# jcyk/gtos

Measured on AMD Instinct MI355X. Metric: graphs/sec training step (100-node AMR, batch 64), higher is better.
Workload: dtype bf16

## Files before the change

gtos_amd/csrc/rel_attn.hip:

```cpp
#include "common.h"
#include "attn_tile.h"
#include <cstdlib>
#include <type_traits>

namespace {

template <typename T> struct Raw8;
template <> struct Raw8<bf16_t> {
    uint4 a;
    __device__ __forceinline__ void load(const bf16_t* p) { a = *reinterpret_cast<const uint4*>(p); }
    __device__ __forceinline__ void zero() { a = make_uint4(0, 0, 0, 0); }
    __device__ __forceinline__ void get(float (&v)[8]) const {
        v[0] = lo_bf(a.x); v[1] = hi_bf(a.x); v[2] = lo_bf(a.y); v[3] = hi_bf(a.y);
        v[4] = lo_bf(a.z); v[5] = hi_bf(a.z); v[6] = lo_bf(a.w); v[7] = hi_bf(a.w);
    }
};
template <> struct Raw8<float> {
    float4 a, b;
    __device__ __forceinline__ void load(const float* p) {
        a = *reinterpret_cast<const float4*>(p); b = *reinterpret_cast<const float4*>(p + 4);
    }
    __device__ __forceinline__ void zero() { a = make_float4(0, 0, 0, 0); b = a; }
    __device__ __forceinline__ void get(float (&v)[8]) const {
        v[0] = a.x; v[1] = a.y; v[2] = a.z; v[3] = a.w; v[4] = b.x; v[5] = b.y; v[6] = b.z; v[7] = b.w;
    }
};

#ifndef GTOS_ATTN_U
#define GTOS_ATTN_U 1
#endif
template <typename T> struct Unroll { static constexpr int U = GTOS_ATTN_U; };
template <> struct Unroll<float> { static constexpr int U = 1; };

struct AttnArgs {
    const void *q, *k, *v; int64_t ldq, ldk, ldv;
    const void* rel;
    const int* idx_q;
    const int* idx_k;
    const uint8_t* key_pad;
    const uint8_t* attn_mask;
    void* o; int64_t ldo;
    float* lse;
    float* w;
    const void* d_o; int64_t lddo;
    const float* dw;
    void *dq, *dk, *dv; int64_t lddq, lddk, lddv;
    int64_t ld_drel;
    void* d_rel;
    float* pd;
    float* gs;
    int T, S, B, H, d, mode;
    int hd, nhs, lr;
    float scale, p_drop; uint64_t seed;
};

struct LaneMap { int LR, g, cl, c, h; bool act, lead; };
template <int LH, bool GEN>
__device__ __forceinline__ LaneMap lane_map(int d, int H, int hd, int nhs, int lr, int lane) {
    LaneMap m;
    if constexpr (!GEN) {
        m.LR = d >> 3; m.g = lane / m.LR; m.cl = lane % m.LR; m.c = m.cl * 8; m.h = m.cl / LH;
        m.act = true; m.lead = (m.cl % LH) == 0;
    } else {
        m.LR = lr; m.g = lane / lr; m.cl = lane % lr;
        const int hl = m.cl / LH, p = m.cl % LH;
        m.h = (int)blockIdx.y * nhs + hl;
        m.c = m.h * hd + p * 8;
        m.act = m.h < H && p * 8 < hd;
        m.lead = m.act && p == 0;
    }
    return m;
}

#define GTOS_DPP(v, ctrl) __builtin_bit_cast(float, __builtin_amdgcn_update_dpp(0, __builtin_bit_cast(int, (v)), (ctrl), 0xF, 0xF, true))
template <int LH> __device__ __forceinline__ float head_sum(float v) {
    if (LH >= 2) v += GTOS_DPP(v, 0xB1);
    if (LH >= 4) v += GTOS_DPP(v, 0x4E);
    if (LH >= 8) v += GTOS_DPP(v, 0x141);
    if (LH >= 16) v += GTOS_DPP(v, 0x140);
    if (LH >= 32) v += __shfl_xor(v, 16);
    if (LH >= 64) v += __shfl_xor(v, 32);
    return v;
}

__device__ __forceinline__ bool map_block(int rows, int B, int& row, int& b) {
    const int blk = blockIdx.x;
    if ((B & 7) == 0) { const int x = blk & 7, w = blk >> 3, gpx = B >> 3; b = x * gpx + (w % gpx); row = w / gpx; }
    else { b = blk % B; row = blk / B; }
    return row < rows;
}

__device__ __forceinline__ bool is_masked(const AttnArgs& a, int i, int j, int b) {
    bool m = false;
    if (a.key_pad) m = a.key_pad[(int64_t)j * a.B + b] != 0;
    if (a.attn_mask) m = m || (a.attn_mask[(int64_t)i * a.S + j] != 0);
    return m;
}

constexpr int MAXS_LDS = 1024;
__device__ __forceinline__ const unsigned char* stage_mask(const AttnArgs& a, int i, int b, unsigned char* sm) {
    const bool use = (a.key_pad || a.attn_mask) && a.S <= MAXS_LDS;
    if (use) for (int j = threadIdx.x; j < a.S; j += 256) sm[j] = is_masked(a, i, j, b) ? 1 : 0;
    __syncthreads();
    return use ? sm : nullptr;
}
__device__ __forceinline__ const int* stage_ids(const int* __restrict__ src, int n, int* sid) {
    if (!src || n > MAXS_LDS) return nullptr;
    for (int j = threadIdx.x; j < n; j += 256) sid[j] = src[j];
    return sid;
}
__device__ __forceinline__ bool key_dead(const AttnArgs& a, const unsigned char* sm, int i, int j, int b) {
    if (sm) return sm[j] != 0;
    return (a.key_pad || a.attn_mask) ? is_masked(a, i, j, b) : false;
}

template <typename T, int LH, bool GEN>
__global__ __launch_bounds__(256, 4) void rel_attn_fwd_kernel(AttnArgs a) {
    if (a.p_drop > 0.f) a.seed = live_seed(a.seed);
    constexpr int U = Unroll<T>::U;
    __shared__ unsigned char smask[MAXS_LDS];
    __shared__ int sid[MAXS_LDS];
    __shared__ float red[4][64][10];
    __shared__ float fin[64][2];
    int i, b;
    if (!map_block(a.T, a.B, i, b)) return;
    const int* sidp = stage_ids(a.mode == 2 ? a.idx_q + ((int64_t)i * a.B + b) * a.S : nullptr, a.S, sid);
    const unsigned char* sm = stage_mask(a, i, b, smask);
    const int lane = threadIdx.x & 63, wv = threadIdx.x >> 6;
    const LaneMap lm = lane_map<LH, GEN>(a.d, a.H, a.hd, a.nhs, a.lr, lane);
    const int d = a.d, LR = lm.LR, G = 64 / LR, g = lm.g, c = lm.c, h = lm.h;
    const bool act = lm.act, lead = lm.lead;
    const int KS = 4 * G;
    const T* qp = static_cast<const T*>(a.q) + ((int64_t)i * a.B + b) * a.ldq + c;
    const T* kb = static_cast<const T*>(a.k) + (int64_t)b * a.ldk + c;
    const T* vb = static_cast<const T*>(a.v) + (int64_t)b * a.ldv + c;
    const T* rel = static_cast<const T*>(a.rel);
    const int* iq = a.mode == 2 ? (sidp ? sidp : a.idx_q + ((int64_t)i * a.B + b) * a.S) : nullptr;
    const float keep_scale = a.p_drop > 0.f ? 1.f / (1.f - a.p_drop) : 1.f;
    const int joff = wv * G + g;

    float qf[8];
    { Raw8<T> r; r.zero(); if (act) r.load(qp); r.get(qf); }
    float m = -INFINITY, l = 0.f, o[8] = {0, 0, 0, 0, 0, 0, 0, 0};

    struct KeySet { Raw8<T> ra[U], rb[U], k[U], v[U]; int tn[U]; };
    auto load_idx = [&](int jb, KeySet& ks) {
#pragma unroll
        for (int u = 0; u < U; ++u) { const int j = jb + u * KS + joff; ks.tn[u] = (iq && j < a.S) ? iq[j] : 0; }
    };
    auto issue = [&](int jb, KeySet& ks) {
#pragma unroll
        for (int u = 0; u < U; ++u) {
            const int j = jb + u * KS + joff;
            ks.ra[u].zero(); ks.rb[u].zero(); ks.k[u].zero(); ks.v[u].zero();
            if (j < a.S && act) {
                ks.k[u].load(kb + (int64_t)j * a.B * a.ldk);
                ks.v[u].load(vb + (int64_t)j * a.B * a.ldv);
                if (a.mode == 1) {
                    const T* p = rel + (((int64_t)j * a.T + i) * a.B + b) * (2 * d) + c;
                    ks.ra[u].load(p); ks.rb[u].load(p + d);
                } else if (a.mode == 2) {
                    const T* p = rel + (int64_t)(ks.tn[u] & 0x7fffffff) * (2 * d) + c;
                    ks.ra[u].load(p); ks.rb[u].load(p + d);
                }
            }
        }
    };
    auto consume = [&](int jb, const KeySet& ks) {
#pragma unroll
        for (int u = 0; u < U; ++u) {
            const int j = jb + u * KS + joff;
            float ra[8], rb[8], kf[8], vf[8];
            ks.ra[u].get(ra); ks.rb[u].get(rb); ks.k[u].get(kf); ks.v[u].get(vf);
            float s = 0.f;
#pragma unroll
            for (int e = 0; e < 8; ++e) s = fmaf(qf[e] + ra[e], kf[e] + rb[e], s);
            s = head_sum<LH>(s) * a.scale;
            const bool dead = (j >= a.S) || key_dead(a, sm, i, j, b);
            if (dead) s = -INFINITY;
            if (a.w && j < a.S && lead) a.w[(((int64_t)i * a.S + j) * a.B + b) * a.H + h] = s;
            const float mn = fmaxf(m, s);
            float alpha = 1.f, pe = 0.f;
            if (mn != -INFINITY) { alpha = __expf(m - mn); pe = __expf(s - mn); }
            l = l * alpha + pe;
            float pv = pe;
            if (a.p_drop > 0.f && !dead)
                pv = drop_keep(a.seed, (((uint64_t)i * a.S + j) * a.B + b) * a.H + h, a.p_drop) ? pe * keep_scale : 0.f;
#pragma unroll
            for (int e = 0; e < 8; ++e) o[e] = fmaf(o[e], alpha, pv * vf[e]);
            m = mn;
        }
    };
    const int STEP = KS * U;
    KeySet A, Bs;
    load_idx(0, A); load_idx(STEP, Bs);
    issue(0, A);
    for (int jb = 0; jb < a.S; jb += 2 * STEP) {
        issue(jb + STEP, Bs); load_idx(jb + 2 * STEP, A);
        consume(jb, A);
        if (jb + STEP >= a.S) break;
        issue(jb + 2 * STEP, A); load_idx(jb + 3 * STEP, Bs);
        consume(jb + STEP, Bs);
    }
    for (int off = LR; off < 64; off <<= 1) {
        const float m2 = __shfl_xor(m, off), l2 = __shfl_xor(l, off);
        const float mn = fmaxf(m, m2);
        float a1 = 1.f, a2 = 1.f;
        if (mn != -INFINITY) { a1 = __expf(m - mn); a2 = __expf(m2 - mn); }
        l = l * a1 + l2 * a2;
#pragma unroll
        for (int e = 0; e < 8; ++e) { const float o2 = __shfl_xor(o[e], off); o[e] = o[e] * a1 + o2 * a2; }
        m = mn;
    }
    red[wv][lane][0] = m; red[wv][lane][1] = l;
#pragma unroll
    for (int e = 0; e < 8; ++e) red[wv][lane][2 + e] = o[e];
    __syncthreads();
    if (wv == 0) {
#pragma unroll
        for (int w2 = 1; w2 < 4; ++w2) {
            const float m2 = red[w2][lane][0], l2 = red[w2][lane][1];
            const float mn = fmaxf(m, m2);
            float a1 = 1.f, a2 = 1.f;
            if (mn != -INFINITY) { a1 = __expf(m - mn); a2 = __expf(m2 - mn); }
            l = l * a1 + l2 * a2;
#pragma unroll
            for (int e = 0; e < 8; ++e) o[e] = o[e] * a1 + red[w2][lane][2 + e] * a2;
            m = mn;
        }
        const float inv = l > 0.f ? 1.f / l : 0.f;
        fin[lane][0] = m; fin[lane][1] = inv;
        if (g == 0 && act) {
            float r[8];
#pragma unroll
            for (int e = 0; e < 8; ++e) r[e] = o[e] * inv;
            Vec8<T>::store(static_cast<T*>(a.o) + ((int64_t)i * a.B + b) * a.ldo + c, r);
            if (lead) a.lse[((int64_t)i * a.B + b) * a.H + h] = (l > 0.f) ? m + __logf(l) : -INFINITY;
        }
    }
    if (a.w) {
        __syncthreads();
        if (lead) {
            const float mf = fin[lane][0], inv = fin[lane][1];
            for (int j = joff; j < a.S; j += KS) {
                const int64_t off = (((int64_t)i * a.S + j) * a.B + b) * a.H + h;
                const float s = a.w[off];
                float p = (s == -INFINITY || inv <= 0.f) ? 0.f : __expf(s - mf) * inv;
                if (a.p_drop > 0.f && p > 0.f) p = drop_keep(a.seed, (uint64_t)off, a.p_drop) ? p * keep_scale : 0.f;
                a.w[off] = p;
            }
        }
    }
}

template <typename T, int LH, bool GEN>
__global__ __launch_bounds__(256) void rel_attn_bwd_q_kernel(AttnArgs a) {
    if (a.p_drop > 0.f) a.seed = live_seed(a.seed);
    constexpr int U = Unroll<T>::U;
    __shared__ unsigned char smask[MAXS_LDS];
    __shared__ int sid[MAXS_LDS];
    __shared__ float red[4][64][8];
    __shared__ float redw[4][64];
    int i, b;
    if (!map_block(a.T, a.B, i, b)) return;
    const int* sidp = stage_ids(a.mode == 2 ? a.idx_q + ((int64_t)i * a.B + b) * a.S : nullptr, a.S, sid);
    const unsigned char* sm = stage_mask(a, i, b, smask);
    const int lane = threadIdx.x & 63, wv = threadIdx.x >> 6;
    const LaneMap lm = lane_map<LH, GEN>(a.d, a.H, a.hd, a.nhs, a.lr, lane);
    const int d = a.d, LR = lm.LR, G = 64 / LR, g = lm.g, c = lm.c, h = lm.h;
    const bool act = lm.act, lead = lm.lead;
    const int KS = 4 * G, joff = wv * G + g;
    const int64_t row = (int64_t)i * a.B + b;
    const T* kb = static_cast<const T*>(a.k) + (int64_t)b * a.ldk + c;
    const T* vb = static_cast<const T*>(a.v) + (int64_t)b * a.ldv + c;
    const T* rel = static_cast<const T*>(a.rel);
    const int* iq = a.mode == 2 ? (sidp ? sidp : a.idx_q + row * a.S) : nullptr;
    const float keep_scale = a.p_drop > 0.f ? 1.f / (1.f - a.p_drop) : 1.f;

    float qf[8], dof[8], of[8];
    { Raw8<T> r; r.zero(); if (act) r.load(static_cast<const T*>(a.q) + row * a.ldq + c); r.get(qf); }
    { Raw8<T> r; r.zero(); if (act) r.load(static_cast<const T*>(a.d_o) + row * a.lddo + c); r.get(dof); }
    { Raw8<T> r; r.zero(); if (act) r.load(static_cast<const T*>(a.o) + row * a.ldo + c); r.get(of); }
    float D = 0.f;
#pragma unroll
    for (int e = 0; e < 8; ++e) D = fmaf(dof[e], of[e], D);
    D = head_sum<LH>(D);
    if (a.dw) {
        float acc = 0.f;
        for (int j = joff; j < a.S && act; j += KS) {
            const int64_t off = (((int64_t)i * a.S + j) * a.B + b) * a.H + h;
            acc = fmaf(a.w[off], a.dw[off], acc);
        }
        for (int off = LR; off < 64; off <<= 1) acc += __shfl_xor(acc, off);
        redw[wv][lane] = acc;
        __syncthreads();
        D += redw[0][lane] + redw[1][lane] + redw[2][lane] + redw[3][lane];
    }
    const float lse = act ? a.lse[row * a.H + h] : -INFINITY;
    float dq[8] = {0, 0, 0, 0, 0, 0, 0, 0};

    struct KeySet { Raw8<T> ra[U], rb[U], k[U], v[U]; int tn[U], tw[U]; };
    auto load_idx = [&](int jb, KeySet& ks) {
#pragma unroll
        for (int u = 0; u < U; ++u) { const int j = jb + u * KS + joff; ks.tn[u] = (iq && j < a.S) ? iq[j] : 0; }
    };
    auto issue = [&](int jb, KeySet& ks) {
#pragma unroll
        for (int u = 0; u < U; ++u) {
            const int j = jb + u * KS + joff;
            ks.ra[u].zero(); ks.rb[u].zero(); ks.k[u].zero(); ks.v[u].zero();
            if (j < a.S && act) {
                ks.k[u].load(kb + (int64_t)j * a.B * a.ldk);
                ks.v[u].load(vb + (int64_t)j * a.B * a.ldv);
                if (a.mode == 1) {
                    const T* p = rel + (((int64_t)j * a.T + i) * a.B + b) * (2 * d) + c;
                    ks.ra[u].load(p); ks.rb[u].load(p + d);
                } else if (a.mode == 2) {
                    const T* p = rel + (int64_t)(ks.tn[u] & 0x7fffffff) * (2 * d) + c;
                    ks.ra[u].load(p); ks.rb[u].load(p + d);
                    ks.tw[u] = ks.tn[u];
                }
            }
        }
    };
    auto consume = [&](int jb, const KeySet& ks) {
#pragma unroll
        for (int u = 0; u < U; ++u) {
            const int j = jb + u * KS + joff;
            if (j >= a.S) continue;
            float ra[8], rb[8], kf[8], vf[8];
            ks.ra[u].get(ra); ks.rb[u].get(rb); ks.k[u].get(kf); ks.v[u].get(vf);
            float s = 0.f, dpv = 0.f;
#pragma unroll
            for (int e = 0; e < 8; ++e) {
                ra[e] += qf[e]; rb[e] += kf[e];
                s = fmaf(ra[e], rb[e], s);
                dpv = fmaf(dof[e], vf[e], dpv);
            }
            s = head_sum<LH>(s) * a.scale;
            dpv = head_sum<LH>(dpv);
            const int64_t off = (((int64_t)i * a.S + j) * a.B + b) * a.H + h;
            const bool dead = key_dead(a, sm, i, j, b) || lse == -INFINITY;
            const float p = dead ? 0.f : __expf(s - lse);
            float keep = 1.f;
            if (a.p_drop > 0.f) keep = drop_keep(a.seed, (uint64_t)off, a.p_drop) ? keep_scale : 0.f;
            float dp = dpv;
            if (a.dw && act) dp += a.dw[off];
            const float gsc = a.scale * p * (keep * dp - D);
            if (lead) { a.pd[off] = p * keep; a.gs[off] = gsc; }
            float dra[8], drb[8];
#pragma unroll
            for (int e = 0; e < 8; ++e) { dra[e] = gsc * rb[e]; drb[e] = gsc * ra[e]; dq[e] += dra[e]; }
            if (!act) {
            } else if (a.mode == 1) {
                T* p2 = static_cast<T*>(a.d_rel) + (((int64_t)j * a.T + i) * a.B + b) * (2 * d) + c;
                Vec8<T>::store(p2, dra);
                Vec8<T>::store(p2 + d, drb);
            } else if (a.mode == 2 && ks.tw[u] < 0 && a.d_rel) {
                T* p2 = static_cast<T*>(a.d_rel) + (int64_t)(ks.tw[u] & 0x7fffffff) * a.ld_drel + c;
                Vec8<T>::store(p2, dra);
                Vec8<T>::store(p2 + d, drb);
            }
        }
    };
    const int STEP = KS * U;
    KeySet A, Bs;
    load_idx(0, A); load_idx(STEP, Bs);
    issue(0, A);
    for (int jb = 0; jb < a.S; jb += 2 * STEP) {
        issue(jb + STEP, Bs); load_idx(jb + 2 * STEP, A);
        consume(jb, A);
        if (jb + STEP >= a.S) break;
        issue(jb + 2 * STEP, A); load_idx(jb + 3 * STEP, Bs);
        consume(jb + STEP, Bs);
    }
    for (int off = LR; off < 64; off <<= 1) {
#pragma unroll
        for (int e = 0; e < 8; ++e) dq[e] += __shfl_xor(dq[e], off);
    }
#pragma unroll
    for (int e = 0; e < 8; ++e) red[wv][lane][e] = dq[e];
    __syncthreads();
    if (wv == 0 && g == 0 && act) {
#pragma unroll
        for (int e = 0; e < 8; ++e) dq[e] = red[0][lane][e] + red[1][lane][e] + red[2][lane][e] + red[3][lane][e];
        Vec8<T>::store(static_cast<T*>(a.dq) + row * a.lddq + c, dq);
    }
}

template <typename T, int LH, bool GEN>
__global__ __launch_bounds__(256) void rel_attn_bwd_kv_kernel(AttnArgs a) {
    constexpr int U = Unroll<T>::U;
    __shared__ float red[4][64][16];
    __shared__ int sid[MAXS_LDS];
    int j, b;
    if (!map_block(a.S, a.B, j, b)) return;
    const int* sidp = stage_ids(a.mode == 2 ? a.idx_k + ((int64_t)j * a.B + b) * a.T : nullptr, a.T, sid);
    if (sidp) __syncthreads();
    const int lane = threadIdx.x & 63, wv = threadIdx.x >> 6;
    const LaneMap lm = lane_map<LH, GEN>(a.d, a.H, a.hd, a.nhs, a.lr, lane);
    const int d = a.d, LR = lm.LR, G = 64 / LR, g = lm.g, c = lm.c, h = lm.h;
    const bool act = lm.act;
    const int KS = 4 * G, ioff = wv * G + g;
    const int64_t row = (int64_t)j * a.B + b;
    const T* qb = static_cast<const T*>(a.q) + (int64_t)b * a.ldq + c;
    const T* dob = static_cast<const T*>(a.d_o) + (int64_t)b * a.lddo + c;
    const T* rel = static_cast<const T*>(a.rel);
    const int* ik = a.mode == 2 ? (sidp ? sidp : a.idx_k + row * a.T) : nullptr;
    float dk[8] = {0, 0, 0, 0, 0, 0, 0, 0}, dv[8] = {0, 0, 0, 0, 0, 0, 0, 0};

    for (int ib = 0; ib < a.T; ib += KS * U) {
        Raw8<T> rq[U], rdo[U], rra[U];
        float pdv[U], gsv[U];
#pragma unroll
        for (int u = 0; u < U; ++u) {
            const int i = ib + u * KS + ioff;
            rq[u].zero(); rdo[u].zero(); rra[u].zero(); pdv[u] = 0.f; gsv[u] = 0.f;
            if (i < a.T && act) {
                rq[u].load(qb + (int64_t)i * a.B * a.ldq);
                rdo[u].load(dob + (int64_t)i * a.B * a.lddo);
                const int64_t off = (((int64_t)i * a.S + j) * a.B + b) * a.H + h;
                pdv[u] = a.pd[off]; gsv[u] = a.gs[off];
                if (a.mode == 1) rra[u].load(rel + (((int64_t)j * a.T + i) * a.B + b) * (2 * d) + c);
                else if (a.mode == 2) rra[u].load(rel + (int64_t)(ik[i] & 0x7fffffff) * (2 * d) + c);
            }
        }
#pragma unroll
        for (int u = 0; u < U; ++u) {
            float qf[8], dof[8], ra[8];
            rq[u].get(qf); rdo[u].get(dof); rra[u].get(ra);
#pragma unroll
            for (int e = 0; e < 8; ++e) { dv[e] = fmaf(pdv[u], dof[e], dv[e]); dk[e] = fmaf(gsv[u], qf[e] + ra[e], dk[e]); }
        }
    }
    for (int off = LR; off < 64; off <<= 1) {
#pragma unroll
        for (int e = 0; e < 8; ++e) { dk[e] += __shfl_xor(dk[e], off); dv[e] += __shfl_xor(dv[e], off); }
    }
#pragma unroll
    for (int e = 0; e < 8; ++e) { red[wv][lane][e] = dk[e]; red[wv][lane][8 + e] = dv[e]; }
    __syncthreads();
    if (wv == 0 && g == 0 && act) {
#pragma unroll
        for (int e = 0; e < 8; ++e) {
            dk[e] = red[0][lane][e] + red[1][lane][e] + red[2][lane][e] + red[3][lane][e];
            dv[e] = red[0][lane][8 + e] + red[1][lane][8 + e] + red[2][lane][8 + e] + red[3][lane][8 + e];
        }
        Vec8<T>::store(static_cast<T*>(a.dk) + row * a.lddk + c, dk);
        Vec8<T>::store(static_cast<T*>(a.dv) + row * a.lddv + c, dv);
    }
}

struct BankArgs {
    const void *q, *k; int64_t ldq, ldk;
    const void* bank; const float* gs;
    const int* pair_sorted;
    const int* chunk_type;
    const int* chunk_start;
    const int* chunk_count;
    const int* chunk_slot;
    const int* xcd_off;
    void* d_bank; int64_t ld_dbank;
    float* heavy;
    int nchunks, T, S, B, H, d;
    int hd, nhs, lr;
};

template <typename T, int LH, bool GEN, int NP>
__global__ __launch_bounds__(256) void rel_attn_bwd_bank_kernel(BankArgs a) {
    const int lane = threadIdx.x & 63;
    const LaneMap lm = lane_map<LH, GEN>(a.d, a.H, a.hd, a.nhs, a.lr, lane);
    const int d = a.d, LR = lm.LR, G = 64 / LR, g = lm.g, c = lm.c, h = lm.h;
    const bool act = lm.act;
    struct Meta { int t, start, cnt, slot; };
    struct Lvl2 { Raw8<T> rRA, rRB; int my_pid; };
    int lo = 0, hi = a.nchunks, stride = gridDim.x * 4, first = blockIdx.x * 4;
    if (a.xcd_off) {
        const int x = blockIdx.x & 7;
        lo = a.xcd_off[x]; hi = a.xcd_off[x + 1];
        stride = (gridDim.x >> 3) * 4; first = lo + (blockIdx.x >> 3) * 4;
    }
    const int last = hi - 1;
    auto load_meta = [&](int ch) {
        const int cc = ch < last ? ch : last;
        Meta m;
        m.t = a.chunk_type[cc]; m.start = a.chunk_start[cc]; m.cnt = a.chunk_count[cc]; m.slot = a.chunk_slot[cc];
        return m;
    };
    auto load_lvl2 = [&](const Meta& m) {
        Lvl2 l;
        const T* bp = static_cast<const T*>(a.bank) + (int64_t)m.t * (2 * d) + c;
        l.rRA.zero(); l.rRB.zero();
        if (act) { l.rRA.load(bp); l.rRB.load(bp + d); }
        l.my_pid = lane < min(m.cnt, 64) ? a.pair_sorted[m.start + lane] : 0;
        return l;
    };
    int ch = first + (threadIdx.x >> 6);
    if (ch >= hi) return;
    Meta m1 = load_meta(ch), m2 = load_meta(ch + stride);
    Lvl2 l1 = load_lvl2(m1);
    for (; ch < hi; ch += stride) {
        const Lvl2 l2 = load_lvl2(m2);
        const Meta m3 = load_meta(ch + 2 * stride);
        const int cnt = m1.cnt;
        float da[8] = {0, 0, 0, 0, 0, 0, 0, 0}, db[8] = {0, 0, 0, 0, 0, 0, 0, 0}, gsum = 0.f;
        for (int sb = 0; sb < cnt; sb += 64) {
            const int nb = min(64, cnt - sb);
            const int my_pid = sb == 0 ? l1.my_pid : (lane < nb ? a.pair_sorted[m1.start + sb + lane] : 0);
            for (int p0 = 0; p0 < nb; p0 += NP * G) {
                Raw8<T> rk[NP], rq[NP];
                float gsc[NP];
#pragma unroll
                for (int u = 0; u < NP; ++u) {
                    const int p = p0 + u * G + g;
                    const int pid = __shfl(my_pid, p < nb ? p : 0);
                    rk[u].zero(); rq[u].zero(); gsc[u] = 0.f;
                    if (p < nb && act) {
                        const int b = pid % a.B, ji = pid / a.B, i = ji % a.T, j = ji / a.T;
                        gsc[u] = a.gs[(((int64_t)i * a.S + j) * a.B + b) * a.H + h];
                        rk[u].load(static_cast<const T*>(a.k) + ((int64_t)j * a.B + b) * a.ldk + c);
                        rq[u].load(static_cast<const T*>(a.q) + ((int64_t)i * a.B + b) * a.ldq + c);
                    }
                }
#pragma unroll
                for (int u = 0; u < NP; ++u) {
                    float kf[8], qf[8];
                    rk[u].get(kf); rq[u].get(qf);
                    gsum += gsc[u];
#pragma unroll
                    for (int e = 0; e < 8; ++e) { da[e] = fmaf(gsc[u], kf[e], da[e]); db[e] = fmaf(gsc[u], qf[e], db[e]); }
                }
            }
        }
        for (int off = LR; off < 64; off <<= 1) {
            gsum += __shfl_xor(gsum, off);
#pragma unroll
            for (int e = 0; e < 8; ++e) { da[e] += __shfl_xor(da[e], off); db[e] += __shfl_xor(db[e], off); }
        }
        if (g == 0 && act) {
            float RA[8], RB[8];
            l1.rRA.get(RA); l1.rRB.get(RB);
            if (m1.slot >= 0) {
                float* out = a.heavy + (int64_t)m1.slot * (2 * d) + c;
#pragma unroll
                for (int e = 0; e < 8; ++e) { atomicAdd(out + e, fmaf(gsum, RB[e], da[e])); atomicAdd(out + d + e, fmaf(gsum, RA[e], db[e])); }
            } else {
                T* out = static_cast<T*>(a.d_bank) + (int64_t)m1.t * a.ld_dbank + c;
                float r1[8], r2[8];
#pragma unroll
                for (int e = 0; e < 8; ++e) { r1[e] = fmaf(gsum, RB[e], da[e]); r2[e] = fmaf(gsum, RA[e], db[e]); }
                Vec8<T>::store(out, r1);
                Vec8<T>::store(out + d, r2);
            }
        }
        m1 = m2; l1 = l2; m2 = m3;
    }
}

template <typename K> int dispatch_lh(int lh, K&& f) {
    switch (lh) {
        case 1: return f(std::integral_constant<int, 1>());
        case 2: return f(std::integral_constant<int, 2>());
        case 4: return f(std::integral_constant<int, 4>());
        case 8: return f(std::integral_constant<int, 8>());
        case 16: return f(std::integral_constant<int, 16>());
        case 32: return f(std::integral_constant<int, 32>());
        case 64: return f(std::integral_constant<int, 64>());
    }
    return -11;
}

struct Geo { int LH, nhs, lr, slices; bool generic; };
int pow2ceil(int x) { int p = 1; while (p < x) p <<= 1; return p; }
int geometry(int d, int H, Geo& g) {
    if (H <= 0 || d <= 0 || d % H) return -10;
    const int hd = d / H;
    if (hd % 8 || hd > 512) return -10;
    g.generic = !(d <= 512 && (d & (d - 1)) == 0 && (hd & (hd - 1)) == 0);
    if (!g.generic) { g.LH = hd / 8; g.nhs = H; g.lr = d / 8; g.slices = 1; return 0; }
    g.LH = pow2ceil(hd / 8);
    int nhs = 64 / g.LH;
    const int hp = pow2ceil(H);
    if (nhs > hp) nhs = hp;
    g.nhs = nhs; g.lr = nhs * g.LH; g.slices = (H + nhs - 1) / nhs;
    return 0;
}
int check_shape(int d, int H) { Geo g; return geometry(d, H, g); }

int nblocks(int rows, int B) { return rows * B; }

}

static int fill_args(AttnArgs& a, Geo& g, int T_, int S, int B, int H, int d, int mode, float scale, float p_drop, uint64_t seed) {
    a.T = T_; a.S = S; a.B = B; a.H = H; a.d = d; a.mode = mode; a.scale = scale; a.p_drop = p_drop; a.seed = seed;
    if (mode != 0 && T_ != S) return -12;
    const int rc = geometry(d, H, g);
    if (rc) return rc;
    a.hd = d / H; a.nhs = g.nhs; a.lr = g.lr;
    return 0;
}

static AttnTileArgs tile_args(const AttnArgs& a) {
    AttnTileArgs t = {};
    t.q = a.q; t.k = a.k; t.v = a.v; t.ldq = a.ldq; t.ldk = a.ldk; t.ldv = a.ldv; t.key_pad = a.key_pad; t.attn_mask = a.attn_mask;
    t.o = a.o; t.ldo = a.ldo; t.lse = a.lse; t.w = a.w; t.d_o = a.d_o; t.lddo = a.lddo; t.dw = a.dw;
    t.dq = a.dq; t.dk = a.dk; t.dv = a.dv; t.lddq = a.lddq; t.lddk = a.lddk; t.lddv = a.lddv;
    t.T = a.T; t.S = a.S; t.B = a.B; t.H = a.H; t.d = a.d; t.scale = a.scale; t.p_drop = a.p_drop; t.seed = a.seed;
    return t;
}

extern "C" int gtos_rel_attn_fwd(int dtype, int mode, int T_, int S, int B, int H, int d,
                                 const void* q, int64_t ldq, const void* k, int64_t ldk, const void* v, int64_t ldv,
                                 const void* rel, const int* idx_q, const uint8_t* key_pad, const uint8_t* attn_mask,
                                 float scale, float p_drop, uint64_t seed,
                                 void* o, int64_t ldo, float* lse, float* w, void* stream) {
    AttnArgs a = {};
    Geo geo;
    int rc = fill_args(a, geo, T_, S, B, H, d, mode, scale, p_drop, seed);
    if (rc) return rc;
    a.q = q; a.k = k; a.v = v; a.ldq = ldq; a.ldk = ldk; a.ldv = ldv; a.rel = rel; a.idx_q = idx_q;
    a.key_pad = key_pad; a.attn_mask = attn_mask; a.o = o; a.ldo = ldo; a.lse = lse; a.w = w;
    if (mode == 0 && dtype == GTOS_BF16 && !geo.generic) {
        const AttnTileArgs t = tile_args(a);
        if (gtosi_attn_tile_covers(T_, S, B, H, d, t, false)) return gtosi_attn_tile_fwd(t, stream);
    }
    hipStream_t s = static_cast<hipStream_t>(stream);
    const dim3 grid(nblocks(T_, B), geo.slices);
    return dispatch_lh(geo.LH, [&](auto lh) {
        constexpr int LH = decltype(lh)::value;
        if (geo.generic) {
            if (dtype == GTOS_BF16) hipLaunchKernelGGL((rel_attn_fwd_kernel<bf16_t, LH, true>), grid, dim3(256), 0, s, a);
            else hipLaunchKernelGGL((rel_attn_fwd_kernel<float, LH, true>), grid, dim3(256), 0, s, a);
        } else {
            if (dtype == GTOS_BF16) hipLaunchKernelGGL((rel_attn_fwd_kernel<bf16_t, LH, false>), grid, dim3(256), 0, s, a);
            else hipLaunchKernelGGL((rel_attn_fwd_kernel<float, LH, false>), grid, dim3(256), 0, s, a);
        }
        GTOS_CHECK_LAUNCH();
        return 0;
    });
}

extern "C" int gtos_rel_attn_bwd(int dtype, int mode, int T_, int S, int B, int H, int d,
                                 const void* q, int64_t ldq, const void* k, int64_t ldk, const void* v, int64_t ldv,
                                 const void* rel, const int* idx_q, const int* idx_k,
                                 const uint8_t* key_pad, const uint8_t* attn_mask,
                                 float scale, float p_drop, uint64_t seed,
                                 const void* o, int64_t ldo, const float* lse, const float* w,
                                 const void* d_o, int64_t lddo, const float* dw,
                                 void* dq, int64_t lddq, void* dk, int64_t lddk, void* dv, int64_t lddv,
                                 void* d_rel, int64_t ld_drel, float* pd, float* gs, void* stream) {
    AttnArgs a = {};
    Geo geo;
    int rc = fill_args(a, geo, T_, S, B, H, d, mode, scale, p_drop, seed);
    if (rc) return rc;
    a.q = q; a.k = k; a.v = v; a.ldq = ldq; a.ldk = ldk; a.ldv = ldv; a.rel = rel; a.idx_q = idx_q; a.idx_k = idx_k;
    a.key_pad = key_pad; a.attn_mask = attn_mask; a.o = const_cast<void*>(o); a.ldo = ldo;
    a.lse = const_cast<float*>(lse); a.w = const_cast<float*>(w); a.d_o = d_o; a.lddo = lddo; a.dw = dw;
    a.dq = dq; a.dk = dk; a.dv = dv; a.lddq = lddq; a.lddk = lddk; a.lddv = lddv; a.d_rel = d_rel; a.ld_drel = ld_drel; a.pd = pd; a.gs = gs;
    if (mode == 2 && d_rel && (ld_drel < 2 * d || ld_drel % 8)) return -14;
    if (dw && !w) return -13;
    if (mode == 0 && dtype == GTOS_BF16 && !geo.generic) {
        const AttnTileArgs t = tile_args(a);
        if (gtosi_attn_tile_covers(T_, S, B, H, d, t, true)) return gtosi_attn_tile_bwd(t, stream);
    }
    if (!pd || !gs) return -15;
    hipStream_t s = static_cast<hipStream_t>(stream);
    const dim3 gq(nblocks(T_, B), geo.slices), gk(nblocks(S, B), geo.slices);
    return dispatch_lh(geo.LH, [&](auto lh) {
        constexpr int LH = decltype(lh)::value;
#define GTOS_BWD(TT, GG) do { hipLaunchKernelGGL((rel_attn_bwd_q_kernel<TT, LH, GG>), gq, dim3(256), 0, s, a); \
                              hipLaunchKernelGGL((rel_attn_bwd_kv_kernel<TT, LH, GG>), gk, dim3(256), 0, s, a); } while (0)
        if (geo.generic) { if (dtype == GTOS_BF16) GTOS_BWD(bf16_t, true); else GTOS_BWD(float, true); }
        else { if (dtype == GTOS_BF16) GTOS_BWD(bf16_t, false); else GTOS_BWD(float, false); }
#undef GTOS_BWD
        GTOS_CHECK_LAUNCH();
        return 0;
    });
}

extern "C" int gtos_rel_attn_bwd_bank(int dtype, int n, int B, int H, int d,
                                      const void* q, int64_t ldq, const void* k, int64_t ldk,
                                      const void* bank, const float* gs,
                                      const int* pair_sorted, const int* chunk_type, const int* chunk_start,
                                      const int* chunk_count, const int* chunk_slot, const int* xcd_off, int nchunks,
                                      void* d_bank, int64_t ld_dbank, float* heavy, void* stream) {
    Geo geo;
    int rc = geometry(d, H, geo);
    if (rc) return rc;
    if (ld_dbank < 2 * d || ld_dbank % 8) return -14;
    if (nchunks <= 0) return 0;
    BankArgs a;
    a.q = q; a.k = k; a.ldq = ldq; a.ldk = ldk; a.bank = bank; a.gs = gs; a.pair_sorted = pair_sorted;
    a.chunk_type = chunk_type; a.chunk_start = chunk_start; a.chunk_count = chunk_count; a.chunk_slot = chunk_slot;
    a.d_bank = d_bank; a.ld_dbank = ld_dbank; a.heavy = heavy; a.nchunks = nchunks; a.T = n; a.S = n; a.B = B; a.H = H; a.d = d;
    a.xcd_off = xcd_off;
    a.hd = d / H; a.nhs = geo.nhs; a.lr = geo.lr;
    hipStream_t s = static_cast<hipStream_t>(stream);
    int grid = (nchunks + 3) / 4; if (grid > 4096) grid = 4096;
    if (xcd_off) grid = (grid + 7) / 8 * 8;
    const dim3 g2(grid, geo.slices);
    return dispatch_lh(geo.LH, [&](auto lh) {
        constexpr int LH = decltype(lh)::value;
        if (geo.generic) {
            if (dtype == GTOS_BF16) hipLaunchKernelGGL((rel_attn_bwd_bank_kernel<bf16_t, LH, true, 4>), g2, dim3(256), 0, s, a);
            else hipLaunchKernelGGL((rel_attn_bwd_bank_kernel<float, LH, true, 4>), g2, dim3(256), 0, s, a);
        } else {
            if (dtype == GTOS_BF16) hipLaunchKernelGGL((rel_attn_bwd_bank_kernel<bf16_t, LH, false, 2>), g2, dim3(256), 0, s, a);
            else hipLaunchKernelGGL((rel_attn_bwd_bank_kernel<float, LH, false, 4>), g2, dim3(256), 0, s, a);
        }
        GTOS_CHECK_LAUNCH();
        return 0;
    });
}

GTOS_SEED_EPOCH_SETTER(rel_attn)
```

Baseline: 857.4.

## Add software-pipelined bf16 relation-bank backward kernel with staged atomics

Adds a new backward kernel for the relation bank gradient. It double-buffers the per-pair k/q/score loads across rows so memory latency overlaps the FMA accumulation, and prefetches chunk metadata and pair ids two chunks ahead. Address arithmetic uses 24-bit multiplies, guarded by a host-side size check. Heavy-slot atomics go through LDS staging so each element gets one atomic per wave instead of one per lane group. This adds register and LDS pressure and code complexity, and is enabled by default for non-generic bf16 shapes with an environment opt-out.

```diff
diff --git a/gtos_amd/csrc/rel_attn.hip b/gtos_amd/csrc/rel_attn.hip
--- a/gtos_amd/csrc/rel_attn.hip
+++ b/gtos_amd/csrc/rel_attn.hip
@@ -557,6 +557,124 @@
     }
 }
 
+template <typename T, int LH, int NP>
+__global__ __launch_bounds__(256, 4) void rel_attn_bwd_bank_pipe_kernel(BankArgs a) {
+    __shared__ float stage[4][2 * 512];
+    const int lane = threadIdx.x & 63;
+    const LaneMap lm = lane_map<LH, false>(a.d, a.H, a.hd, a.nhs, a.lr, lane);
+    const int d = a.d, LR = lm.LR, G = 64 / LR, g = lm.g, c = lm.c, h = lm.h;
+    const int per = NP * G;
+    struct Meta { int t, start, cnt, slot; };
+    struct Rows { Raw8<T> rk[NP], rq[NP]; float gsc[NP]; };
+    int lo = 0, hi = a.nchunks, stride = gridDim.x * 4, first = blockIdx.x * 4;
+    if (a.xcd_off) {
+        const int x = blockIdx.x & 7;
+        lo = a.xcd_off[x]; hi = a.xcd_off[x + 1];
+        stride = (gridDim.x >> 3) * 4; first = lo + (blockIdx.x >> 3) * 4;
+    }
+    const int last = hi - 1;
+    auto load_meta = [&](int ch) {
+        const int cc = ch < last ? ch : last;
+        Meta m;
+        m.t = a.chunk_type[cc]; m.start = a.chunk_start[cc]; m.cnt = a.chunk_count[cc]; m.slot = a.chunk_slot[cc];
+        return m;
+    };
+    auto uni = [](const Meta& m) {
+        Meta u;
+        u.t = __builtin_amdgcn_readfirstlane(m.t); u.start = __builtin_amdgcn_readfirstlane(m.start);
+        u.cnt = __builtin_amdgcn_readfirstlane(m.cnt); u.slot = __builtin_amdgcn_readfirstlane(m.slot);
+        return u;
+    };
+    auto load_pids = [&](const Meta& m) { return lane < min(m.cnt, 64) ? a.pair_sorted[m.start + lane] : 0; };
+    const char* const qb = static_cast<const char*>(a.q);
+    const char* const kb = static_cast<const char*>(a.k);
+    const char* const gb = reinterpret_cast<const char*>(a.gs);
+    const uint32_t qrow = (uint32_t)a.ldq * sizeof(T), krow = (uint32_t)a.ldk * sizeof(T), hrow = a.H * 4, cb = c * sizeof(T), hb = h * 4;
+    auto mad24 = [](uint32_t x, uint32_t y, uint32_t z) { return __umul24(x, y) + z; };
+    int ch = first + (threadIdx.x >> 6);
+    if (ch >= hi) return;
+    Meta m1 = uni(load_meta(ch)), m2v = load_meta(ch + stride);
+    int pid1 = load_pids(m1);
+    for (; ch < hi; ch += stride) {
+        const Meta m2 = uni(m2v);
+        const int pid2 = load_pids(m2);
+        Raw8<T> rRA, rRB;
+        {
+            const T* bp = static_cast<const T*>(a.bank) + (int64_t)m1.t * (2 * d) + c;
+            rRA.load(bp); rRB.load(bp + d);
+        }
+        m2v = load_meta(ch + 2 * stride);
+        const int cnt = m1.cnt, pend = m1.start + cnt - 1;
+        float da[8] = {0, 0, 0, 0, 0, 0, 0, 0}, db[8] = {0, 0, 0, 0, 0, 0, 0, 0}, gsum = 0.f;
+        int my_pid = pid1;
+        for (int sb = 0; sb < cnt; sb += 64) {
+            const int nb = min(64, cnt - sb), R = (nb + per - 1) / per;
+            const int nxt_pid = a.pair_sorted[min(m1.start + sb + 64 + lane, pend)];
+            auto issue = [&](Rows& w, int r) {
+#pragma unroll
+                for (int u = 0; u < NP; ++u) {
+                    const int p = r * per + u * G + g;
+                    const int pid = __shfl(my_pid, p < nb ? p : 0);
+                    const uint32_t b = (uint32_t)pid % (uint32_t)a.B, ji = (uint32_t)pid / (uint32_t)a.B, i = ji % (uint32_t)a.T, j = ji / (uint32_t)a.T;
+                    w.gsc[u] = *reinterpret_cast<const float*>(gb + mad24(mad24(mad24(i, a.S, j), a.B, b), hrow, hb));
+                    w.rk[u].load(reinterpret_cast<const T*>(kb + mad24(mad24(j, a.B, b), krow, cb)));
+                    w.rq[u].load(reinterpret_cast<const T*>(qb + mad24(mad24(i, a.B, b), qrow, cb)));
+                }
+                __builtin_amdgcn_sched_barrier(0);
+            };
+            auto consume = [&](const Rows& w, int r) {
+#pragma unroll
+                for (int u = 0; u < NP; ++u) {
+                    float kf[8], qf[8];
+                    w.rk[u].get(kf); w.rq[u].get(qf);
+                    const float gv = r * per + u * G + g < nb ? w.gsc[u] : 0.f;
+                    gsum += gv;
+#pragma unroll
+                    for (int e = 0; e < 8; ++e) { da[e] = fmaf(gv, kf[e], da[e]); db[e] = fmaf(gv, qf[e], db[e]); }
+                }
+#pragma unroll
+                for (int e = 0; e < 8; ++e) asm volatile("" : "+v"(da[e]), "+v"(db[e]));
+                __builtin_amdgcn_sched_barrier(0);
+            };
+            Rows ra, rb;
+            int r = 0;
+            issue(ra, 0);
+            for (; r + 2 < R; r += 2) {
+                issue(rb, r + 1); consume(ra, r);
+                issue(ra, r + 2); consume(rb, r + 1);
+            }
+            if (r + 1 < R) { issue(rb, r + 1); consume(ra, r); consume(rb, r + 1); }
+            else consume(ra, r);
+            my_pid = nxt_pid;
+        }
+        for (int off = LR; off < 64; off <<= 1) {
+            gsum += __shfl_xor(gsum, off);
+#pragma unroll
+            for (int e = 0; e < 8; ++e) { da[e] += __shfl_xor(da[e], off); db[e] += __shfl_xor(db[e], off); }
+        }
+        {
+            float RA[8], RB[8], r1[8], r2[8];
+            rRA.get(RA); rRB.get(RB);
+#pragma unroll
+            for (int e = 0; e < 8; ++e) { r1[e] = fmaf(gsum, RB[e], da[e]); r2[e] = fmaf(gsum, RA[e], db[e]); }
+            if (m1.slot >= 0) {
+                float* st = stage[threadIdx.x >> 6];
+                if (g == 0) {
+#pragma unroll
+                    for (int e = 0; e < 8; ++e) { st[c + e] = r1[e]; st[d + c + e] = r2[e]; }
+                }
+                float* out = a.heavy + (int64_t)m1.slot * (2 * d);
+                for (int f = lane; f < 2 * d; f += 64) atomicAdd(out + f, st[f]);
+            } else if (g == 0) {
+                T* out = static_cast<T*>(a.d_bank) + (int64_t)m1.t * a.ld_dbank + c;
+                Vec8<T>::store(out, r1);
+                Vec8<T>::store(out + d, r2);
+            }
+        }
+        m1 = m2; pid1 = pid2;
+    }
+}
+
 template <typename K> int dispatch_lh(int lh, K&& f) {
     switch (lh) {
         case 1: return f(std::integral_constant<int, 1>());
@@ -699,9 +817,14 @@
     int grid = (nchunks + 3) / 4; if (grid > 4096) grid = 4096;
     if (xcd_off) grid = (grid + 7) / 8 * 8;
     const dim3 g2(grid, geo.slices);
+    static const bool use_pipe = !(getenv("GTOS_BANK_PIPE") && getenv("GTOS_BANK_PIPE")[0] == '0');
+    const int64_t n2B = (int64_t)n * n * B, rowq = ldq * 2, rowk = ldk * 2, lim24 = 1 << 24, lim32 = (int64_t)1 << 32;
+    const bool pipe_fits = n2B < lim24 && rowq < lim24 && rowk < lim24 && n2B * H * 4 < lim32 && (int64_t)n * B * rowq < lim32 && (int64_t)n * B * rowk < lim32;
     return dispatch_lh(geo.LH, [&](auto lh) {
         constexpr int LH = decltype(lh)::value;
-        if (geo.generic) {
+        if (!geo.generic && dtype == GTOS_BF16 && use_pipe && pipe_fits) {
+            hipLaunchKernelGGL((rel_attn_bwd_bank_pipe_kernel<bf16_t, LH, 2>), g2, dim3(256), 0, s, a);
+        } else if (geo.generic) {
             if (dtype == GTOS_BF16) hipLaunchKernelGGL((rel_attn_bwd_bank_kernel<bf16_t, LH, true, 4>), g2, dim3(256), 0, s, a);
             else hipLaunchKernelGGL((rel_attn_bwd_bank_kernel<float, LH, true, 4>), g2, dim3(256), 0, s, a);
         } else {
```

Result: no change. 864.1 (median of 6 runs) (+0.8%).
